# cggos/ptam_cg

Hardware: AMD Instinct MI355X
Metric: BA LM iterations/s (50 KF x 5k pts) [+ tracked frames/s @640x480 in 'tracking'] (higher is better)
Workload: dtype f64

## Files before the change

### ptam_cg_amd/csrc/ba_schur.inc

```
__device__ __forceinline__ void vinv_body(const BaDev& d, double lambda, int bx) {
    const int p = bx * 256 + threadIdx.x;
    if (p >= d.P) return;
    double v[6];
    const int r0 = d.rowptr[p], r1 = d.rowptr[p + 1];
    const int c0 = r0 >> 6, c1 = (r1 - 1) >> 6;
    if (d.cut != nullptr && r1 > r0 && c0 != c1) {
        const double* q = d.cut + (size_t)(2 * c0 + 1) * 9;
        double e[3] = {q[6], q[7], q[8]};
#pragma unroll
        for (int i = 0; i < 6; i++) v[i] = q[i];
        for (int c = c0 + 1; c <= c1; c++) {
            q = d.cut + (size_t)(2 * c) * 9;
#pragma unroll
            for (int i = 0; i < 6; i++) v[i] += q[i];
#pragma unroll
            for (int i = 0; i < 3; i++) e[i] += q[6 + i];
        }
#pragma unroll
        for (int i = 0; i < 3; i++) d.epsB[(size_t)p * 3 + i] = e[i];
    } else {
#pragma unroll
        for (int i = 0; i < 6; i++) v[i] = d.V[(size_t)p * 6 + i];
    }
    double A[9] = {v[0], v[1], v[3], v[1], v[2], v[4], v[3], v[4], v[5]};
    double* out = d.Vinv + (size_t)p * 9;
    if (A[0] * A[4] * A[8] == 0) {
#pragma unroll
        for (int i = 0; i < 9; i++) out[i] = 0;
        return;
    }
    A[0] *= (1.0 + lambda);
    A[4] *= (1.0 + lambda);
    A[8] *= (1.0 + lambda);
    for (int col = 0; col < 3; col++) {
        double inv_diag = 1;
        for (int row = col; row < 3; row++) {
            double val = A[row * 3 + col];
            for (int c2 = 0; c2 < col; c2++) val -= A[c2 * 3 + col] * A[row * 3 + c2];
            if (row == col) {
                A[row * 3 + col] = val;
                inv_diag = 1 / val;
            } else {
                A[col * 3 + row] = val;
                A[row * 3 + col] = val * inv_diag;
            }
        }
    }
    for (int c = 0; c < 3; c++) {
        double y[3], x[3];
        for (int i = 0; i < 3; i++) {
            double val = (i == c) ? 1.0 : 0.0;
            for (int j = 0; j < i; j++) val -= A[i * 3 + j] * y[j];
            y[i] = val;
        }
        for (int i = 0; i < 3; i++) y[i] /= A[i * 3 + i];
        for (int i = 2; i >= 0; i--) {
            double val = y[i];
            for (int j = i + 1; j < 3; j++) val -= A[j * 3 + i] * x[j];
            x[i] = val;
        }
        for (int r = 0; r < 3; r++) out[r * 3 + c] = x[r];
    }
}

__global__ void __launch_bounds__(256) vinv_kernel(BaDev d, double lambda) {
    TL_MARK(d, 6)
    if (ba_guard_blocks(d)) return;
    vinv_body(d, lambda, blockIdx.x);
}
__global__ void __launch_bounds__(256) reduce_vinv_kernel(BaDev d, int grid_acc, int nx, double lambda, double lambda_stay) {
    TL_MARK(d, 5)
    const int4 gf = ba_guard_load(d);
    if (ba_guard_blocks(d, gf)) return;
    if (ba_guard_stay(d, gf)) lambda = lambda_stay;
    const int b = blockIdx.x, nr = nx * RSPLIT;
    if (b < nr)
        reduce_partials_body(d, grid_acc, b % nx, b / nx);
    else
        vinv_body(d, lambda, b - nr);
}

#define SCHUR_TILE_ELEMS (SCHUR_TC * SCHUR_TC * 36 + SCHUR_TC * 6)
#ifndef SCHUR_RING
#define SCHUR_RING 2
#endif
#ifndef SCHUR_NW
#define SCHUR_NW 4
#endif
#define SCHUR_WG_PER_CU (8 / SCHUR_NW)
#define SCHUR_RED_BYTES ((SCHUR_NW / 2) * 40 * 64 * 8)
#define SCHUR_N_VARIANTS 6
#define SCHUR_MAP_WPT 8

struct SchurGrp {
    double wa[3][3];
    double wb[3][3];
    double vi[9];
    double eb[3];
    unsigned pm;
};
typedef double v4f64 __attribute__((ext_vector_type(4)));
typedef double schur_d2 __attribute__((ext_vector_type(2), aligned(8)));

template <int MODE>
__host__ __device__ __forceinline__ int schur_row(int t, int rid) {
    if (MODE == 1) return rid;
    if (t < 2) return 6 * (rid / 3) + 2 * (rid % 3) + t;
    const int q = 16 + (rid >> 1);
    return 6 * (q / 3) + 2 * (q % 3) + (rid & 1);
}
struct SchurLane {
    int hi4, sh4, hi2, sh2;
    unsigned o4, o2;
};
template <int MODE>
__device__ __forceinline__ SchurLane schur_lane(int l15) {
    SchurLane L;
    const int r0 = schur_row<MODE>(0, l15), r2 = MODE == 3 ? schur_row<3>(2, l15) : 0;
    const int s0 = r0 / 6, s2 = r2 / 6;
    L.hi4 = s0 >> 2, L.sh4 = 8 * (s0 & 3), L.o4 = 8u * (unsigned)(r0 - 6 * s0);
    L.hi2 = s2 >> 2, L.sh2 = 8 * (s2 & 3), L.o2 = 8u * (unsigned)(r2 - 6 * s2);
    return L;
}

__device__ __forceinline__ unsigned schur_slot_off(unsigned o0, unsigned o1, int first, int hi, int sh, int M, bool& present) {
    const unsigned o = ((hi ? o1 : o0) >> sh) & 0xffu;
    present = o != 0xffu;
    return (present ? (unsigned)first + o : (unsigned)M) * 48u;
}

template <int MODE>
__device__ __forceinline__ void schur_fetch_role(const char* __restrict__ W0, const char* __restrict__ W1, const char* __restrict__ W2,
                                                 unsigned o0, unsigned o1, int first, const SchurLane& L, int M, double w[3][3],
                                                 bool& pres01, bool& pres2) {
    pres2 = false;
    const unsigned off4 = schur_slot_off(o0, o1, first, L.hi4, L.sh4, M, pres01) + L.o4;
#ifdef SCHUR_NOLOAD
    for (int t = 0; t < 3; t++) w[t][0] = w[t][1] = w[t][2] = (double)off4;
    return;
#endif
    if (MODE == 1) {
        w[0][0] = *(const double*)(W0 + off4);
        w[0][1] = *(const double*)(W1 + off4);
        w[0][2] = *(const double*)(W2 + off4);
        return;
    }
    const double2 p0 = *(const double2*)(W0 + off4), p1 = *(const double2*)(W1 + off4), p2 = *(const double2*)(W2 + off4);
    w[0][0] = p0.x, w[1][0] = p0.y;
    w[0][1] = p1.x, w[1][1] = p1.y;
    w[0][2] = p2.x, w[1][2] = p2.y;
    if (MODE == 3) {
        const unsigned off2 = schur_slot_off(o0, o1, first, L.hi2, L.sh2, M, pres2) + L.o2;
#ifdef SCHUR_NOFRAG2
        w[2][0] = w[2][1] = w[2][2] = (double)off2;
        return;
#endif
        w[2][0] = *(const double*)(W0 + off2);
        w[2][1] = *(const double*)(W1 + off2);
        w[2][2] = *(const double*)(W2 + off2);
    }
}

// ... 315 lines not shown
    std::vector<unsigned> dev((size_t)SCHUR_N_VARIANTS * NT * SCHUR_MAP_WPT, 0xffffffffu);
    for (int v = 0; v < SCHUR_N_VARIANTS; v++)
        for (int t = 0; t < NT; t++)
            for (int i = 0; i < SCHUR_MAP_WPT && t + NT * i < NE2; i++) {
                const int e = t + NT * i;
                dev[((size_t)v * NT + t) * SCHUR_MAP_WPT + i] = (unsigned)m[(size_t)v * SCHUR_TILE_ELEMS + 2 * e] | ((unsigned)m[(size_t)v * SCHUR_TILE_ELEMS + 2 * e + 1] << 16);
            }
    return dev;
}

__global__ void __launch_bounds__(64 * SCHUR_NW) __attribute__((amdgpu_waves_per_eu(2, 2))) schur_tile_mfma_kernel(BaDev d) {
    TL_MARK(d, 7)
    extern __shared__ __attribute__((aligned(16))) double red[];
#ifdef SCHUR_STAMPS
    const long long t_entry = (long long)__builtin_amdgcn_s_memtime();
    if (threadIdx.x == 0 && blockIdx.x < 512) {
        unsigned hw, xcc;
        asm volatile("s_getreg_b32 %0, hwreg(HW_REG_HW_ID)" : "=s"(hw));
        asm volatile("s_getreg_b32 %0, hwreg(HW_REG_XCC_ID)" : "=s"(xcc));
        d.dbg[3072 + 2 * blockIdx.x] = ((long long)__builtin_amdgcn_s_memrealtime() & ((1ll << 40) - 1)) | ((long long)((xcc & 0xf) << 16 | (hw & 0xffff)) << 40);
    }
#endif
#ifdef SCHUR_NO_HEAD
    const int sg0 = d.s_wg_seg[blockIdx.x], sg1 = d.s_wg_seg[blockIdx.x + 1];
#else
    const int4 h0 = ((const int4*)d.s_wg_head)[2 * blockIdx.x], h1 = ((const int4*)d.s_wg_head)[2 * blockIdx.x + 1];
    const int sg0 = h0.x, sg1 = h0.y;
#endif
    for (int sg = sg0; sg < sg1; sg++) {
#ifdef SCHUR_NO_HEAD
        const SchurWG wg = d.s_segs[sg];
#else
        const SchurWG wg = sg == sg0 ? SchurWG{h0.z, h0.w, h1.x, h1.y} : d.s_segs[sg];
#endif
        int a = (int)((sqrt(8.0 * wg.pair + 1.0) - 1.0) * 0.5);
        while ((a + 1) * (a + 2) / 2 <= wg.pair) a++;
        while (a * (a + 1) / 2 > wg.pair) a--;
        const int b = wg.pair - a * (a + 1) / 2;
        const int ncam = min(SCHUR_TC, d.F - a * SCHUR_TC);
        const int ma = ncam <= 2 ? 1 : (ncam <= 5 ? 2 : 3);
        if (a == b) {
            if (ma == 3) schur_tile_body<true, 3, 3>(d, wg, red);
            else if (ma == 2) schur_tile_body<true, 2, 2>(d, wg, red);
            else schur_tile_body<true, 1, 1>(d, wg, red);
        } else {
            if (ma == 3) schur_tile_body<false, 3, 3>(d, wg, red);
            else if (ma == 2) schur_tile_body<false, 2, 3>(d, wg, red);
            else schur_tile_body<false, 1, 3>(d, wg, red);
        }
        __syncthreads();
    }
#ifdef SCHUR_STAMPS
    if (threadIdx.x == 0 && blockIdx.x < 512) d.dbg[3072 + 2 * blockIdx.x + 1] = (long long)__builtin_amdgcn_s_memrealtime() | ((long long)(sg1 - sg0) << 56);
    if ((blockIdx.x == 0 || blockIdx.x == 150) && threadIdx.x == 0) {
        long long* o = d.dbg + 2048 + (blockIdx.x ? 512 : 0) + 264;
        o[0] = t_entry, o[1] = (long long)__builtin_amdgcn_s_memtime(), o[2] = sg1 - sg0;
    }
#endif
}

#define SRED_SLICES 10
__device__ __forceinline__ double schur_sum_partials(const double* __restrict__ elem, int w0, int w1) {
#ifdef SRED_NOLOAD
    return (double)(w1 - w0);
#endif
    double s0 = 0, s1 = 0, s2 = 0, s3 = 0;
    for (int w = w0; w < w1; w += 32) {
        double q[32];
#pragma unroll
        for (int i = 0; i < 32; i++) {
            const double v = elem[(size_t)min(w + i, w1 - 1) * SCHUR_TILE_ELEMS];
            q[i] = w + i < w1 ? v : 0.0;
        }
#pragma unroll
        for (int i = 0; i < 32; i += 4) {
            s0 += q[i];
            s1 += q[i + 1];
            s2 += q[i + 2];
            s3 += q[i + 3];
        }
    }
    return (s0 + s1) + (s2 + s3);
}
__global__ void __launch_bounds__(256) schur_reduce_kernel(BaDev d, double lambda, int pad_identity) {
    TL_MARK(d, 8)
    const int pair = blockIdx.x, slice = blockIdx.y;
    int a = (int)((sqrt(8.0 * pair + 1.0) - 1.0) * 0.5);
    while ((a + 1) * (a + 2) / 2 <= pair) a++;
    while (a * (a + 1) / 2 > pair) a--;
    const int b = pair - a * (a + 1) / 2;
    const int wg0 = d.s_pair_wg_begin[pair], wg1 = d.s_pair_wg_begin[pair + 1];
    double* S = d.SE;
    double* E = se_E(d);
    const int band = se_band(d);
    const size_t FS = (size_t)d.F * 27;
    if (slice < 9) {
        const int idx = slice * 256 + threadIdx.x;
        const int jk = idx / 36, rc = idx - jk * 36;
        const int j = jk >> 3, k = jk & 7, r = rc / 6, c = rc - r * 6;
        const int fa = a * SCHUR_TC + j, fb = b * SCHUR_TC + k;
        if (fa >= d.F || fb >= d.F) return;
        if (a == b && j < k) return;
        const int Rr = 6 * fa + r, Cc = 6 * fb + c, Rb = Rr / SOLVE_NB, Cb = Cc / SOLVE_NB;
        if (Cb > Rb || Rb - Cb > band) return;
        const bool dg = a == b && j == k;
        const int rr = r >= c ? r : c, cc = r >= c ? c : r;
        double uq[RSPLIT];
#pragma unroll
        for (int sp = 0; sp < RSPLIT; sp++) uq[sp] = dg ? d.Usplit[sp * FS + fa * 27 + rr * (rr + 1) / 2 + cc] : 0.0;
        const double tsum = schur_sum_partials(d.s_part + idx, wg0, wg1);
        double val = -tsum;
        if (dg) {
            double u = 0;
#pragma unroll
            for (int sp = 0; sp < RSPLIT; sp++) u += uq[sp];
            if (r == c) u *= (1.0 + lambda);
            val += u;
        }
        S[se_blk(Rb, Cb, band) + (size_t)(Rr % SOLVE_NB) * SOLVE_NB + (Cc % SOLVE_NB)] = val;
        return;
    }
    if (a == b && threadIdx.x < SCHUR_TC * 6) {
        const int idx = threadIdx.x;
        const int j = idx / 6, r = idx - j * 6;
        const int fa = a * SCHUR_TC + j;
        if (fa < d.F) {
            const double s = schur_sum_partials(d.s_part + SCHUR_TC * SCHUR_TC * 36 + idx, wg0, wg1);
            double ea = 0;
#pragma unroll
            for (int sp = 0; sp < RSPLIT; sp++) ea += d.Usplit[sp * FS + fa * 27 + 21 + r];
            E[6 * fa + r] = ea - s;
        }
    }
    {
        const int np = d.npad - d.n, total = np * d.npad;
        for (int idx = pair * 256 + threadIdx.x; idx < total; idx += 256 * (int)gridDim.x) {
            const int q = idx / d.npad;
            const int r = d.n + q, c = idx - q * d.npad;
            const int Rb = r / SOLVE_NB, Cb = c / SOLVE_NB;
            if (c <= r && Rb - Cb <= band)
                S[se_blk(Rb, Cb, band) + (size_t)(r % SOLVE_NB) * SOLVE_NB + (c % SOLVE_NB)] = (r == c && pad_identity) ? 1.0 : 0.0;
        }
    }
    if (pair == 0) {
        const int np = d.npad - d.n;
        for (int idx = threadIdx.x; idx < np; idx += 256) E[d.n + idx] = 0.0;
    }
}
```

### ptam_cg_amd/csrc/bundle.h

```cpp
#pragma once
#include <cstddef>

#include "common.h"

enum { MS_ALIVE = 0, MS_BAD = 1, MS_DEAD = 2 };

#define BA_CHUNK 256
#define SCHUR_TC 8
#define SOLVE_NB 32
#define HIST_BINS 4096

struct BaChunk {
    int pt_begin, pt_end, m_begin, m_end;
};

struct SchurEntry {
    int pt;
    int ma;
    int mb;
    int pad;
    unsigned offa[2];
    unsigned offb[2];
};
struct SchurWG {
    int pair;
    int e_begin, e_end;
    int slot;
};

struct BaScalars {
    double sigma_sq;
    double cur_err;
    double new_err;
    double sumsq_cam;
    double sumsq_pt;
    double median;
    long long n_valid;
    int n_bad;
    int n_outliers;
    int sel_bin;
    int sel_k;
    int n_cand;
    int sel_bin2;
    int sel_k2;
    int select_overflow;
    int n_outliers_pub;
    int pad_;
    int end_step;
    int spec_go;
    int spec_stay;
    int spec_seq;
    int abort_any;
    int solve_fault;
};
static_assert(offsetof(BaScalars, end_step) % 16 == 0 && sizeof(BaScalars) % 8 == 0, "BaScalars: the decision words are read as one 16-byte load");

struct BaDev {
    int C, F, P, M;
    int guard;
    int guard_seq;
    int n, npad;
    int band;
    int n_chunks, grid_acc;
    int u_rows;
    int n_wchunks;
    int n_tiles, n_pairs, n_schur_wg, n_schur_entries;
    double* pose[2];
    int* cam_free;
    double* pt[2];
    double* V;
    double* epsB;
    double* Vinv;
    double* cut;
    int* rowptr;
    int* m_cam;
    int* m_pt;
    double2* m_found;
    double* m_s;
    int* m_orig;
    int* m_fidx;
    uint8_t* m_state;
    double* m_e2;
    double* m_e2t;
    uint8_t* m_zbad_t;
    double* W;
    double* Usplit;
    double* Upart;
    double* Adet;
    int* cam_ptr;
    int* cam_meas;
    double* err_part;
    int* bad_part;
    BaChunk* chunks;
    BaChunk* wchunks;
    unsigned* hist;
    double* cand;
    SchurEntry* s_entries;
    SchurWG* s_segs;
    int* s_wg_seg;
    int* s_pair_wg_begin;
    int* s_wg_head;
    double* s_part;
    unsigned* s_map;
    double* SE;
    double* L;
    double* Dg;
    double* y;
    double* da;
    double *SE2, *L2, *Dg2, *y2;
    unsigned* sflags2;
    unsigned* sflags;
    unsigned solve_seq;
    int chain_off;
    int chain_xcd;
    int spin_limit;
    double* bw_scratch;
    double* sumsq2;
    int* outliers;
    BaScalars* sc;
    long long* dbg;
};

__host__ __device__ __forceinline__ size_t w_plane(const BaDev& d) { return (size_t)(d.M + 1) * 6; }

__host__ __device__ __forceinline__ size_t se_blocks_before_row(int bi, int band) {
    return bi <= band ? (size_t)bi * (bi + 1) / 2 : (size_t)(band + 1) * (band + 2) / 2 + (size_t)(bi - band - 1) * (band + 1);
}
__host__ __device__ __forceinline__ size_t se_blk(int bi, int bj, int band) {
    const int j0 = bi - band > 0 ? bi - band : 0;
    return (se_blocks_before_row(bi, band) + (size_t)(bj - j0)) * (SOLVE_NB * SOLVE_NB);
}
__host__ __device__ __forceinline__ size_t se_size(int nblk, int band) { return se_blocks_before_row(nblk, band) * (SOLVE_NB * SOLVE_NB); }
__host__ __device__ __forceinline__ int se_band(const BaDev& d) {
    const int nblk = d.npad / SOLVE_NB;
    return d.band < nblk - 1 ? d.band : (nblk > 0 ? nblk - 1 : 0);
}
__host__ __device__ __forceinline__ double* se_E(const BaDev& d) { return d.SE + se_size(d.npad / SOLVE_NB, se_band(d)); }

#define MS_LOG 15
#define MS_CH (1 << MS_LOG)
#define MS_CH_BYTES ((size_t)MS_CH * 32)
template <class B>
__host__ __device__ __forceinline__ B* ms_chunk(B* base, size_t i) { return base + (i >> MS_LOG) * MS_CH_BYTES; }
__host__ __device__ __forceinline__ const int& ms_cam(const char* base, size_t i) { return ((const int*)ms_chunk(base, i))[i & (MS_CH - 1)]; }
__host__ __device__ __forceinline__ const int& ms_pt(const char* base, size_t i) { return ((const int*)(ms_chunk(base, i) + (size_t)MS_CH * 4))[i & (MS_CH - 1)]; }
__host__ __device__ __forceinline__ const double2& ms_found(const char* base, size_t i) { return ((const double2*)(ms_chunk(base, i) + (size_t)MS_CH * 8))[i & (MS_CH - 1)]; }
__host__ __device__ __forceinline__ const double& ms_sig(const char* base, size_t i) { return ((const double*)(ms_chunk(base, i) + (size_t)MS_CH * 24))[i & (MS_CH - 1)]; }

struct Carver {
    size_t off = 0;
    size_t take(size_t bytes) {
        const size_t o = off;
        off += (bytes + 255) & ~(size_t)255;
        return o;
    }
// ... 36 lines not shown
```

### ptam_cg_amd/csrc/bundle.hip

```cpp
#include <algorithm>
#include <array>
#include <chrono>
#include <climits>
#include <atomic>
#include <numeric>
#include <utility>

#include "bundle.h"
#include "../../include/ptam_hip_bench.h"

#include "ba_math.inc"
#include "ba_pass1.inc"
#include "ba_select.inc"
#include "ba_jacobian.inc"
#include "ba_schur.inc"
#include "ba_update.inc"
#include "ba_prepare.inc"

template <class T>
struct PinVec {
    ptam_ctx* ctx = nullptr;
    T* p = nullptr;
    size_t n = 0, cap = 0, cap_bytes = 0;
    size_t size() const { return n; }
// ... 365 lines not shown
    const int n_cu = ctx->n_cu > 0 ? ctx->n_cu : 256;
    auto k7_fn = [&](int threads) -> const void* { return k7_wave_fn(threads, ba->k7_loop, ba->opts.estimator, ba->k7_big, ba->det); };
    auto k7_occupancy = [&](int threads, int* per_cu) -> int { return ba_k7_occupancy(ctx, k7_fn(threads), threads, k7_smem(threads), per_cu); };
    int per_cu = 0;
    {
        const size_t lds_max = 160 * 1024;
        if (k7_smem(ba->k7_threads) > lds_max) {
            for (int t : {512, 256})
                if (k7_smem(t) <= lds_max) {
                    ba->k7_threads = t;
                    break;
                }
            if (k7_smem(ba->k7_threads) > lds_max) {
                ba->k7_big = true;
                ba->k7_loop = true;
                ba->k7_threads = 256;
            }
        }
        if (ba->det && !ba->k7_big && ba->k7_threads != (ba->k7_loop ? 256 : 1024)) {
            ba->k7_loop = true;
            ba->k7_threads = 256;
        }
    }
    if (int rc = k7_occupancy(ba->k7_threads, &per_cu)) {
        ptam_set_error("the accumulation kernel cannot be launched with %zu bytes of LDS (%d free cameras)", k7_smem(ba->k7_threads), F);
        return rc;
    }
    if (ba->k7_loop && !ba->k7_big && !ba->det) {
        for (int t : {512, 1024}) {
            int per_cu_t = 0;
            if (int rc = k7_occupancy(t, &per_cu_t)) return rc;
            if (per_cu_t * t > per_cu * ba->k7_threads) {
                ba->k7_threads = t;
                per_cu = per_cu_t;
            }
        }
    }
    per_cu = std::max(1, std::min(per_cu, 8));
    if (ba->use_wave && ba->k7_loop && !ba->k7_big) {
        if (const char* e = ptam_ab_env("PTAM_K7_THREADS")) {
            const int t = atoi(e);
            if ((t == 256 || t == 512 || t == 1024) && !(ba->det && t != 256) && k7_smem(t) <= 160 * 1024) {
                ba->k7_threads = t;
                if (int rc = k7_occupancy(t, &per_cu)) return rc;
                per_cu = std::max(1, std::min(per_cu, 8));
            }
        }
        if (const char* e = ptam_ab_env("PTAM_K7_WG_PER_CU")) per_cu = std::max(1, std::min(per_cu, atoi(e)));
    }
    if (ba->use_wave && !ba->k7_loop) {
        if (const char* e = ptam_ab_env("PTAM_K7_THREADS1")) {
            const int t = atoi(e);
            if ((t == 512 || t == 1024) && !(ba->det && t != 1024) && k7_smem(t) <= 160 * 1024) {
                ba->k7_threads = t;
                if (int rc = k7_occupancy(t, &per_cu)) return rc;
            }
        }
    }
    ba->smem_acc = k7_smem(ba->k7_threads);
    if (ba->use_wave) {
        const int n64 = (M + 63) / 64;
        const int wpb = ba->k7_threads / 64;
        if (ba->k7_loop) {
            d.grid_acc = std::max(1, std::min(n_cu * per_cu, n64 / wpb));
            const int waves = d.grid_acc * wpb;
            ba->per_wave = n64 / waves;
            ba->extra_waves = n64 - ba->per_wave * waves;
        } else {
            ba->per_wave = 1;
            ba->extra_waves = 0;
            d.grid_acc = std::max(1, (n64 + wpb - 1) / wpb);
        }
    } else
        d.grid_acc = 1;
    const int n_dtiles = (M + DET_TILE - 1) / DET_TILE;
    d.u_rows = ba->det ? n_dtiles : (ba->k7_big || !ba->use_wave) ? 1 : d.grid_acc;
    lap("launch shape");

    Carver cv;
    const size_t Mz = std::max(M, 1), Pz = std::max(P_all, 1), Cz = std::max(C, 1), Fz = std::max(F, 1), Maz = std::max(Mall, 1);
    const size_t chunks_cap = std::min<size_t>(Pz, (size_t)M / 64 + (size_t)P_all / 128 + 8);
    const size_t o_pose0 = cv.take(Cz * 96), o_pose1 = cv.take(Cz * 96);
    const size_t o_pt0 = cv.take(Pz * 24), o_pt1 = cv.take(Pz * 24), o_V = cv.take(Pz * 48), o_epsB = cv.take(Pz * 24),
                 o_Vinv = cv.take(Pz * 72), o_rowptr = cv.take((Pz + 1) * 4),
                 o_cut = cv.take(ba->use_wave ? (size_t)((M + 63) / 64) * 2 * 72 : 8);
    const size_t o_mcam = cv.take(Mz * 4), o_mpt = cv.take(Mz * 4), o_mfound = cv.take(Mz * 16), o_ms = cv.take(Mz * 8),
                 o_morig = cv.take(Mz * 4), o_mfidx = cv.take(Mz * 4), o_mstate = cv.take(Mz), o_me2 = cv.take(Mz * 8), o_me2t = cv.take(Mz * 8), o_zbad = cv.take(Mz), o_W = cv.take((Mz + 1) * 144);
    const size_t o_U = cv.take(Fz * 27 * 8 * 16), o_Upart = cv.take((size_t)std::max(d.grid_acc, ba->det ? n_dtiles : 1) * Fz * 27 * 8);
    const size_t o_adet = cv.take(ba->det ? Mz * 14 * 8 : 8), o_camptr = cv.take(ba->det ? (size_t)n_dtiles * (Fz + 1) * 4 : 8), o_cammeas = cv.take(ba->det ? Mz * 4 : 8),
                 o_tilefree = cv.take(ba->det ? ((size_t)n_dtiles + 1) * 4 : 8);
    const size_t n_part = std::max<size_t>(chunks_cap, (size_t)d.grid_acc);
    const size_t o_errp = cv.take(n_part * 16 + 16), o_badp = cv.take((size_t)d.grid_acc * 4 + 16);
    const size_t o_chunks = cv.take(chunks_cap * sizeof(BaChunk));
    const size_t o_wchunks = cv.take(sizeof(BaChunk));
    const size_t o_hist = cv.take(2 * HIST_BINS * 4), o_cand = cv.take(Mz * 8);
    const size_t npad = std::max(d.npad, SOLVE_NB);
    const size_t se_full = se_size((int)(npad / SOLVE_NB), (int)(npad / SOLVE_NB) - 1);
    const size_t o_SE = cv.take((se_full + npad + 8) * 8), o_L = cv.take(se_full * 8), o_Dg = cv.take(npad * 8),
                 o_y = cv.take(npad * 8), o_da = cv.take(npad * 8), o_sq2 = cv.take(16),
                 o_bws = cv.take(npad * 8 * 12), o_sflags = cv.take(ba_solve_flag_bytes((int)(npad / SOLVE_NB))),
                 o_sflags2 = cv.take(ba_solve_flag_bytes((int)(npad / SOLVE_NB))), o_SE2 = cv.take((se_full + npad + 8) * 8),
                 o_L2 = cv.take(se_full * 8), o_Dg2 = cv.take(npad * 8), o_y2 = cv.take(npad * 8);
    const size_t o_out = cv.take(Mz * 4), o_sc = cv.take(sizeof(BaScalars)), o_dbg = cv.take(65536), o_xchg = cv.take(4096);
    const int nw = std::max(1, (n_tiles + 31) / 32);
    const size_t hist_n = (size_t)8 * std::max(n_pairs, 1) * 16;
    const size_t o_cnt = cv.take(Pz * 4), o_tcode = cv.take(Pz * (size_t)nw * 8), o_phist = cv.take(hist_n * 4);
    const size_t clear_bytes = cv.off;
    Carver sm;
    const size_t s_ps = sm.take(sizeof(PrepScalars)), s_pose = sm.take(Cz * 96), s_camfree = sm.take(Cz * 4),
                 s_porder = sm.take(pair_order.size() * 4);
    const size_t o_small = cv.take(sm.off);
    const size_t o_rdead = cv.take(Maz), o_ptsraw = cv.take(Pz * 24);
    const size_t o_start = cv.take((Pz + 1) * 4), o_denseof = cv.take(Pz * 4), o_ptorig = cv.take(Pz * 4), o_arr = cv.take(Maz * 4),
                 o_tmpi = cv.take(Mz * 4), o_tmpkey = cv.take(Mz * 4), o_ptile = cv.take(Mz * 16), o_kp = cv.take(Pz * 4),
                 o_costp = cv.take(Pz * 4), o_entpre = cv.take((Pz + 1) * 8), o_costpre = cv.take((Pz + 1) * 8), o_ebase = cv.take(hist_n * 4);
    ba->block_bytes = cv.off;
    if (!ctx_cache_take(ctx->dev_cache, CTX_NCACHE(ctx->dev_cache), ba->block_bytes, &ba->block, &ba->block_cap)) {
        HIP_TRY(hipMalloc(&ba->block, ba->block_bytes));
        ba->block_cap = ba->block_bytes;
    }
    HIP_TRY(hipMemsetAsync(ba->block, 0, clear_bytes, ctx->stream));
    char* base = (char*)ba->block;
    d.pose[0] = (double*)(base + o_small + s_pose);
    d.pose[1] = (double*)(base + o_pose1);
    (void)o_pose0;
    d.cam_free = (int*)(base + o_small + s_camfree);
    d.pt[0] = (double*)(base + o_pt0);
    d.pt[1] = (double*)(base + o_pt1);
    d.V = (double*)(base + o_V);
    d.epsB = (double*)(base + o_epsB);
    d.Vinv = (double*)(base + o_Vinv);
    d.cut = ba->use_wave ? (double*)(base + o_cut) : nullptr;
    d.rowptr = (int*)(base + o_rowptr);
    d.m_cam = (int*)(base + o_mcam);
    d.m_pt = (int*)(base + o_mpt);
    d.m_found = (double2*)(base + o_mfound);
    d.m_s = (double*)(base + o_ms);
    d.m_orig = (int*)(base + o_morig);
    d.m_fidx = (int*)(base + o_mfidx);
    d.m_state = (uint8_t*)(base + o_mstate);
    d.m_e2 = (double*)(base + o_me2);
    d.m_e2t = (double*)(base + o_me2t);
    d.m_zbad_t = (uint8_t*)(base + o_zbad);
    d.W = (double*)(base + o_W);
    d.Usplit = (double*)(base + o_U);
    d.Upart = (double*)(base + o_Upart);
    d.Adet = ba->det ? (double*)(base + o_adet) : nullptr;
    d.cam_ptr = (int*)(base + o_camptr);
    d.cam_meas = (int*)(base + o_cammeas);
    d.err_part = (double*)(base + o_errp);
    d.bad_part = (int*)(base + o_badp);
    d.chunks = (BaChunk*)(base + o_chunks);
    d.wchunks = (BaChunk*)(base + o_wchunks);
    d.hist = (unsigned*)(base + o_hist);
    d.cand = (double*)(base + o_cand);
    d.SE = (double*)(base + o_SE);
    d.L = (double*)(base + o_L);
    d.Dg = (double*)(base + o_Dg);
    d.y = (double*)(base + o_y);
    d.da = (double*)(base + o_da);
    d.sumsq2 = (double*)(base + o_sq2);
    d.bw_scratch = (double*)(base + o_bws);
    d.sflags = (unsigned*)(base + o_sflags);
    d.sflags2 = (unsigned*)(base + o_sflags2);
    d.SE2 = (double*)(base + o_SE2);
    d.L2 = (double*)(base + o_L2);
    d.Dg2 = (double*)(base + o_Dg2);
    d.y2 = (double*)(base + o_y2);
    d.solve_seq = 0;
    d.chain_off = 0;
    {
        static std::atomic<unsigned> next_xcd{0};
        d.chain_xcd = (int)(next_xcd.fetch_add(1) & 7u);
        static const int lim = [] {
            const char* e = getenv("PTAM_CH_SPIN_LIMIT");
            return e ? std::max(1, atoi(e)) : CH_SPIN_DEFAULT;
        }();
        d.spin_limit = lim;
    }
    d.outliers = (int*)(base + o_out);
    d.sc = (BaScalars*)(base + o_sc);
    d.dbg = (long long*)(base + o_dbg);
    ba->d_xchg = (double*)(base + o_xchg);
    if (!ctx->d_smap) {
        static const std::vector<unsigned> s_map = schur_index_map_device();
        HIP_TRY(hipMalloc((void**)&ctx->d_smap, s_map.size() * 4));
        HIP_TRY(hipMemcpy(ctx->d_smap, s_map.data(), s_map.size() * 4, hipMemcpyHostToDevice));
    }
    d.s_map = ctx->d_smap;
    lap("alloc + clear");

    Carver hs;
    const size_t h_stamp = hs.take(64), h_psrb = hs.take(sizeof(PrepScalars)), h_rowptr = hs.take((Pz + 1) * 4), h_ptorig = hs.take(Pz * 4),
                 h_small = hs.take(sm.off), h_chunks = hs.take(chunks_cap * sizeof(BaChunk)), h_dead = hs.take(ba->n_dead > 0 ? Maz : 1);
    (void)h_stamp;
    void* pin = nullptr;
    {
        const size_t later = 64 + (size_t)C * 96 + (size_t)P_all * 24 + (size_t)M * 4 + 64;
        const int rc_p = ctx_pinned(ctx, std::max(hs.off, later), &pin);
        if (rc_p) return rc_p;
    }
    char* hp = (char*)pin;
    char* dp = (char*)ctx->d_pinned;
    volatile unsigned long long* stamp = (volatile unsigned long long*)hp;
    PrepScalars* ps_host = (PrepScalars*)(hp + h_psrb);
    {
        PrepScalars init;
        std::memset(&init, 0, sizeof init);
        init.dup_key = ~0ull;
        std::memcpy(hp + h_small + s_ps, &init, sizeof init);
        std::memcpy(hp + h_small + s_pose, ba->cam_pose.data(), (size_t)C * 96);
        std::memcpy(hp + h_small + s_camfree, cam_free.data(), (size_t)C * 4);
        std::memcpy(hp + h_small + s_porder, pair_order.data(), pair_order.size() * 4);
    }
// ... 341 lines not shown
        }
        HIP_TRY(hipMemsetAsync(ba->d_gather, 0, (size_t)total * 8, ctx->stream));
        if (n_local > 0)
            hipLaunchKernelGGL(place_keys_kernel, dim3((n_local + 255) / 256), dim3(256), 0, ctx->stream,
                               (const double*)d.cand, n_local, ba->d_gather + off);
        rc = ba_allreduce(ba, ba->d_gather, (size_t)total);
        if (rc) return rc;
        BaDev dg = d;
        dg.cand = ba->d_gather + ba->gather_cap;
        if (total > 0)
            hipLaunchKernelGGL(hist_keys_kernel, dim3((int)std::max<long long>(1, std::min<long long>((total + 255) / 256, 1024))),
                               dim3(256), 0, ctx->stream, (const double*)ba->d_gather, total, d.hist);
        hipLaunchKernelGGL(select_compact_kernel, dim3((int)std::max<long long>(1, std::min<long long>((total + 1023) / 1024, 256))),
                           dim3(256), 0, ctx->stream, dg, (const double*)ba->d_gather, total, (const uint8_t*)nullptr, 0);
        hipLaunchKernelGGL(select_final_kernel, dim3(1), dim3(1024), 0, ctx->stream, dg, ba->opts.estimator, min_s2);
        prof_end(ba, PTAM_K_SELECT);
        HIP_TRY(hipGetLastError());
        return PTAM_OK;
    }
    hipLaunchKernelGGL(select_final_kernel, dim3(1), dim3(1024), 0, ctx->stream, d, ba->opts.estimator, min_s2);
    prof_end(ba, PTAM_K_SELECT);
    HIP_TRY(hipGetLastError());
    return PTAM_OK;
}

static void launch_k7(ptam_ba* ba, int guard = 0) {
    ptam_ctx* ctx = ba->ctx;
    BaDev d = ba->d;
    d.guard = guard;
    d.guard_seq = (int)ba->mbox_seq;
    int cur = guard ? (ba->cur ^ 1) : ba->cur;
    if ((ba->k7_big && !ba->det) || !ba->use_wave)
        (void)hipMemsetAsync(d.Upart, 0, std::max<size_t>(1, (size_t)d.F * 27) * sizeof(double), ctx->stream);
    if (!ba->use_wave) {
        (void)hipMemsetAsync(d.err_part, 0, 16, ctx->stream);
        (void)hipMemsetAsync(d.bad_part, 0, 4, ctx->stream);
        return;
    }
    int est = ba->opts.estimator;
    void* args[] = {&ctx->cam, &d, &cur, &est, &ba->per_wave, &ba->extra_waves};
    (void)hipLaunchKernel(k7_wave_fn(ba->k7_threads, ba->k7_loop, est, ba->k7_big, ba->det), dim3(d.grid_acc), dim3(ba->k7_threads), args,
                          ba->smem_acc, ctx->stream);
    if (ba->det && d.F > 0)
        hipLaunchKernelGGL(reduce_det_kernel, dim3(d.u_rows), dim3(256), (size_t)14 * (DET_TILE + 1) * sizeof(double), ctx->stream, d);
}

static int ba_pass2(ptam_ba* ba) {
    ptam_ctx* ctx = ba->ctx;
    BaDev& d = ba->d;
    prof_begin(ba, PTAM_K_JACOBIAN);
    launch_k7(ba);
    prof_end(ba, PTAM_K_JACOBIAN);
    hipLaunchKernelGGL(reduce_partials_kernel, dim3(std::max(1, (d.F * 27 + 63) / 64), RSPLIT), dim3(256), 0, ctx->stream,
                       d, d.grid_acc);
    HIP_TRY(hipGetLastError());
    if (ba->comm && ba->world > 1) {
        if (d.F > 0) {
            hipLaunchKernelGGL(pack2_kernel, dim3(1), dim3(1), 0, ctx->stream, (const BaScalars*)d.sc, se_E(d) + d.npad, 0, 0);
            ba->cur_pending = true;
        } else {
            hipLaunchKernelGGL(pack2_kernel, dim3(1), dim3(1), 0, ctx->stream, (const BaScalars*)d.sc, ba->d_xchg, 0, 0);
            int rc = ba_allreduce(ba, ba->d_xchg, 2);
            if (rc) return rc;
            hipLaunchKernelGGL(unpack2_kernel, dim3(1), dim3(1), 0, ctx->stream, d.sc, (const double*)ba->d_xchg, 0);
        }
    }
    return PTAM_OK;
}

static int ba_ensure_mailbox(ptam_ba* ba) {
    if (ba->mbox) return PTAM_OK;
    void* h = nullptr;
    size_t cap = 0;
    if (!ctx_cache_take(ba->ctx->host_cache, CTX_NCACHE(ba->ctx->host_cache), sizeof(ptam_ba::Mailbox), &h, &cap))
        HIP_TRY(hipHostMalloc(&h, sizeof(ptam_ba::Mailbox), hipHostMallocMapped | hipHostMallocCoherent));
    std::memset(h, 0, sizeof(ptam_ba::Mailbox));
    void* dv = nullptr;
    HIP_TRY(hipHostGetDevicePointer(&dv, h, 0));
    ba->mbox = (ptam_ba::Mailbox*)h;
    ba->mbox_dev = (ptam_ba::Mailbox*)dv;
    return PTAM_OK;
}

static int ba_trial(ptam_ba* ba, double lambda, bool skip_vinv, int last_allowed, int abort_local, bool decide_in_prologue = false) {
    ptam_ctx* ctx = ba->ctx;
    BaDev& d = ba->d;
    prof_begin(ba, PTAM_K_VINV);
    if (d.P > 0 && !skip_vinv) hipLaunchKernelGGL(vinv_kernel, dim3((d.P + 255) / 256), dim3(256), 0, ctx->stream, d, lambda);
    prof_end(ba, PTAM_K_VINV);
    if (d.F > 0) {
        prof_begin(ba, PTAM_K_SCHUR);
        if (d.n_schur_wg > 0)
            hipLaunchKernelGGL(schur_tile_mfma_kernel, dim3(d.n_schur_wg), dim3(64 * SCHUR_NW), SCHUR_RED_BYTES, ctx->stream, d);
        hipLaunchKernelGGL(schur_reduce_kernel, dim3(d.n_pairs, SRED_SLICES), dim3(256), 0, ctx->stream, d, lambda,
                           (ba->world > 1 && ba->rank != 0) ? 0 : 1);
        prof_end(ba, PTAM_K_SCHUR);
        HIP_TRY(hipGetLastError());
        const size_t n_se = se_size(d.npad / SOLVE_NB, se_band(d)) + d.npad;
        const bool sharded = ba->comm && ba->world > 1;
        if (sharded) prof_begin(ba, PTAM_K_EXCHANGE);
        int rc = ba_allreduce(ba, d.SE, n_se + (ba->cur_pending ? 2 : 0));
        if (sharded) prof_end(ba, PTAM_K_EXCHANGE);
        if (rc) return rc;
        if (ba->cur_pending) {
            hipLaunchKernelGGL(unpack2_kernel, dim3(1), dim3(1), 0, ctx->stream, d.sc, (const double*)(d.SE + n_se), 0);
            ba->cur_pending = false;
        }
        prof_begin(ba, PTAM_K_SOLVE);
        rc = ba_solve(ctx, d, ba->cur);
        prof_end(ba, PTAM_K_SOLVE);
        if (rc) return rc;
    }
    prof_begin(ba, PTAM_K_UPDATE);
    if (d.F == 0)
        hipLaunchKernelGGL(pose_update_kernel, dim3(std::max(1, (d.C + 63) / 64)), dim3(64), 0, ctx->stream, d, ba->cur);
    if (d.n_chunks > 0)
        hipLaunchKernelGGL(point_update_kernel, dim3(d.n_chunks), dim3(BA_CHUNK), 0, ctx->stream, ctx->cam, d, ba->cur,
                           ba->opts.estimator);
    {
        const bool fuse = !(ba->comm && ba->world > 1) && !ba->prof;
        ulonglong2* slots = nullptr;
        unsigned long long seq = 0;
        if (fuse) {
            const int rcm = ba_ensure_mailbox(ba);
            if (rcm) return rcm;
            slots = (ulonglong2*)ba->mbox_dev;
            seq = ++ba->mbox_seq;
            ba->published_by_finalize = true;
        }
        ba->decide_pending = decide_in_prologue;
        ba->decide_last_allowed = last_allowed;
        if (!decide_in_prologue)
            hipLaunchKernelGGL(finalize_new_kernel, dim3(1), dim3(256), 0, ctx->stream, d, ba->opts.update_sq_conv_limit, last_allowed,
                               slots, seq);
    }
    prof_end(ba, PTAM_K_UPDATE);
    HIP_TRY(hipGetLastError());
    if (ba->comm && ba->world > 1) {
        hipLaunchKernelGGL(pack2_kernel, dim3(1), dim3(1), 0, ctx->stream, (const BaScalars*)d.sc, ba->d_xchg, 1, abort_local);
        int rc = ba_allreduce(ba, ba->d_xchg, 4);
        if (rc) return rc;
        hipLaunchKernelGGL(unpack2_kernel, dim3(1), dim3(1), 0, ctx->stream, d.sc, (const double*)ba->d_xchg, 1);
    }
    return PTAM_OK;
}

static int ba_p1_blocks() {
    static const int n = [] {
        const char* e = ptam_ab_env("PTAM_P1_BLOCKS");
        return e ? std::max(1, atoi(e)) : 512;
    }();
    return n;
}
static int ba_enqueue_speculative(ptam_ba* ba, double lambda_next, double lambda_stay) {
    ptam_ctx* ctx = ba->ctx;
    BaDev d = ba->d;
    const double min_s2 = ba->opts.min_sigma * ba->opts.min_sigma;
    d.guard = 1;
    d.guard_seq = (int)ba->mbox_seq;
    const dim3 g_p1(std::max(1, std::min((d.M + 256 * P1_U - 1) / (256 * P1_U), ba_p1_blocks())));
    if (ba->decide_pending) {
        hipLaunchKernelGGL(purge_pass1_decide_kernel, g_p1, dim3(256), 0, ctx->stream, d, ba->opts.update_sq_conv_limit, ba->decide_last_allowed,
                           (ulonglong2*)ba->mbox_dev, ba->mbox_seq);
        ba->decide_pending = false;
    } else
        hipLaunchKernelGGL(purge_pass1_kernel, g_p1, dim3(256), 0, ctx->stream, d);
    hipLaunchKernelGGL(select_compact_kernel, dim3(std::max(1, std::min((d.M + 1023) / 1024, ba_sel_blocks()))), dim3(256), 0, ctx->stream, d,
                       (const double*)d.m_e2, (long long)d.M, (const uint8_t*)d.m_state, 0);
    hipLaunchKernelGGL(select_final_kernel, dim3(1), dim3(1024), 0, ctx->stream, d, ba->opts.estimator, min_s2);
    launch_k7(ba, 1);
    {
        const int nx = std::max(1, (d.F * 27 + 63) / 64);
        hipLaunchKernelGGL(reduce_vinv_kernel, dim3(nx * RSPLIT + (d.P + 255) / 256), dim3(256), 0, ctx->stream, d, d.grid_acc, nx,
                           lambda_next, lambda_stay);
    }
    HIP_TRY(hipGetLastError());
    return PTAM_OK;
}
// ... 359 lines not shown
        }
        ba->ev_ok = true;
    }
    ba->prof = on != 0;
    return PTAM_OK;
}

int ptam_ba_kernel_time(const ptam_ba* ba, int kernel, double* total_ms, int* launches) {
    ARG_TRY(ba && kernel >= 0 && kernel < PTAM_K_COUNT);
    if (total_ms) *total_ms = ba->k_ms[kernel];
    if (launches) *launches = ba->k_n[kernel];
    return PTAM_OK;
}

int ptam_ba_set_comm(ptam_ba* ba, int rank, int world, ptam_allreduce_f64_fn fn, void* user) {
    ARG_TRY(ba && world >= 1 && rank >= 0 && rank < world);
    ARG_TRY(world == 1 || fn);
    ARG_TRY(world <= 32);
    if (ba->d_sel && world != ba->world) {
        HIP_TRY(hipSetDevice(ba->ctx->device));
        HIP_TRY(ptam_stream_wait(ba->ctx->stream));
        HIP_TRY(hipFree(ba->d_sel));
        ba->d_sel = nullptr;
    }
    ba->rank = rank;
    ba->world = world;
    ba->comm = fn;
    ba->comm_user = user;
    return PTAM_OK;
}

#define BA_DBG(...) do { if (dbg.wait) { std::fprintf(stderr, "[ptam] " __VA_ARGS__); std::fprintf(stderr, "\n"); } } while (0)
int ptam_ba_compute(ptam_ba* ba, const volatile unsigned char* abort_flag, int* accepted_out) {
    ARG_TRY(ba);
    ptam_ctx* ctx = ba->ctx;
    const BaDebug& dbg = ba_debug();
    HIP_TRY(hipSetDevice(ctx->device));
    BA_DBG("compute: prepare");
    const bool sharded = ba->comm && ba->world > 1;
    int rc = ptam_ba_prepare(ba);
    if (rc && !sharded) return rc;
    const int rc_prepare = rc;
    BA_DBG("compute: prepared M=%d P=%d F=%d chunks=%d wchunks=%d grid_acc=%d schur_wg=%d", ba->d.M, ba->d.P, ba->d.F, ba->d.n_chunks,
           ba->d.n_wchunks, ba->d.grid_acc, ba->d.n_schur_wg);
    BaDev& d = ba->d;
    ChainTurn chain_turn(d, ctx->device);
    double lambda = 0.0001, lambda_factor = 2.0;
    ba->converged = ba->published_by_finalize = ba->cur_pending = ba->slow_select = false;
    ba->trial_is_current = ba->e2_is_current = false;
    bool hit_max = false;
    int counter = 0;
    ba->accepted = 0;
    ba->trials.clear();
    std::vector<int> step_outlier_end;
    int n_steps = 0;
    bool prev_end_pending = false;
    bool abort_all = false;
    auto abort_local = [&]() { return abort_flag && *abort_flag; };
    auto aborted = [&]() { return sharded ? abort_all : abort_local(); };
    BaScalars sc;
    std::memset(&sc, 0, sizeof sc);
    double dbg_enq_ms = 0, dbg_wait_ms = 0;
    std::vector<double> trial_read_us;
    const auto dbg_t0 = std::chrono::steady_clock::now();
    BaHostTimes ht;
    ba_dbg_begin(ba, ht);
    if (sharded && (rc = ba_sharded_handshake(ba, rc_prepare, abort_local(), &abort_all, chain_turn))) return rc;
    const bool empty = d.M == 0;
    const bool spec = !sharded && !ba->prof && d.n_chunks > 0 && !ptam_ab_env("PTAM_NO_SPECULATION");
    bool spec_ready = false;
    const bool fused_decision = !ptam_ab_env("PTAM_SEPARATE_FINALIZE");
    while (!empty && !ba->converged && !hit_max && !aborted()) {
        bool skip_vinv = false;
        if (spec_ready) {
            spec_ready = false;
            skip_vinv = true;
        } else {
            if ((rc = ba_pass1_sigma(ba))) return rc;
            if ((rc = ba_pass2(ba))) return rc;
        }
        bool have_cur = false;
        double cur_err = 0, new_err = 0;
        bool ran_any = false, redo_step = false, nan_stop = false;
        for (;;) {
            if (have_cur && !(new_err > cur_err)) break;
            if (ba->converged || hit_max || aborted()) break;
            BA_DBG("trial %d lambda %g", counter, lambda);
            const auto q0 = std::chrono::steady_clock::now();
            rc = ba_trial(ba, lambda, skip_vinv, counter + 1 >= ba->opts.max_iterations ? 1 : 0, abort_local() ? 1 : 0, spec && fused_decision);
            dbg_enq_ms += ba_stall_ms(q0, counter, "took", "to enqueue");
            skip_vinv = false;
            if (rc) return rc;
            if ((rc = ba_publish_scalars(ba))) return rc;
            if (spec) {
                if ((rc = ba_enqueue_speculative(ba, lambda * 0.3, lambda))) return rc;
            }
            BA_DBG("trial %d enqueued, waiting", counter);
            const auto w0 = std::chrono::steady_clock::now();
            rc = ba_wait_scalars(ba, &sc);
            dbg_wait_ms += ba_stall_ms(w0, counter, "waited", "for its scalars");
            if (rc) return rc;
            BA_DBG("trial %d read: cur %g new %g sigma2 %g median %g n_valid %lld n_bad %d sumsq %g %g", counter, sc.cur_err, sc.new_err,
                   sc.sigma_sq, sc.median, sc.n_valid, sc.n_bad, sc.sumsq_cam, sc.sumsq_pt);
            ba_dbg_first_read(ht);
            if (!have_cur) {
                if (prev_end_pending) step_outlier_end.push_back(spec && fused_decision ? sc.n_outliers_pub : sc.n_outliers);
                prev_end_pending = false;
                if (sc.select_overflow && !ba->slow_select) {
                    ba->slow_select = true;
                    if (dbg.select) std::fprintf(stderr, "[ptam] rank %d: select overflow, repeating the step on the gather path\n", ba->rank);
                    redo_step = true;
                    break;
                }
                have_cur = true;
                cur_err = sc.cur_err;
                new_err = cur_err + 9999;
                if (!(new_err > cur_err)) {
                    nan_stop = true;
                    break;
                }
            }
            if (sc.solve_fault) {
                if ((rc = ba_solve_fallback(ba, counter))) return rc;
                continue;
            }
            ran_any = true;
            if (dbg.trial_times) trial_read_us.push_back(std::chrono::duration<double, std::micro>(std::chrono::steady_clock::now() - dbg_t0).count());
            if (sharded) abort_all = abort_all || sc.abort_any != 0;
            new_err = sc.new_err;
            const double sumsq = sc.sumsq_cam + sc.sumsq_pt;
            if (sumsq < ba->opts.update_sq_conv_limit) ba->converged = true;
            ptam_ba_trial t;
            t.lambda = lambda;
            t.sigma_sq = sc.sigma_sq;
            t.err_old = cur_err;
            t.err_new = new_err;
            t.sum_sq_update = sumsq;
            t.n_bad = sc.n_bad;
            t.accepted = 0;
            if (ba->opts.verbose)
                std::printf("L%.1e\tOld %.6f  New %.6f  Diff %.6f\n", lambda, cur_err, new_err, cur_err - new_err);
            if (new_err > cur_err) {
                lambda = lambda * lambda_factor;
                lambda_factor = lambda_factor * 2;
            }
            counter++;
            if (counter >= ba->opts.max_iterations) hit_max = true;
            ba->trials.push_back(t);
        }
        if (redo_step) continue;
        if (nan_stop) hit_max = true;
        ba->trial_is_current = false;
        ba->e2_is_current = ran_any && !(new_err < cur_err);
        if (ran_any && new_err < cur_err) {
            lambda_factor = 2.0;
            lambda *= 0.3;
            ba->cur ^= 1;
            ba->accepted++;
            ba->trials.back().accepted = 1;
            ba->trial_is_current = true;
        }
        if (prev_end_pending) {
            if ((rc = ba_read_scalars(ba, &sc))) return rc;
            step_outlier_end.push_back(sc.n_outliers);
        }
        const bool stayed = spec && ran_any && !(new_err < cur_err) && !(new_err > cur_err) && !ba->converged && !hit_max;
        spec_ready = (spec && ran_any && new_err < cur_err && !ba->converged && !hit_max) || stayed;
        if (!spec_ready && d.M > 0)
            hipLaunchKernelGGL(purge_kernel, dim3((d.M + 255) / 256), dim3(256), 0, ctx->stream, d);
        prev_end_pending = true;
        HIP_TRY(hipGetLastError());
        n_steps++;
    }
    BA_DBG("loop done, steps %d", n_steps);
    ba_report_trial_times(ba, trial_read_us);
    if (dbg.stall)
        std::fprintf(stderr, "[ptam] compute loop: %zu trials in %.3f ms; host enqueueing trials %.3f ms, waiting for scalars %.3f ms\n",
                     ba->trials.size(), std::chrono::duration<double, std::milli>(std::chrono::steady_clock::now() - dbg_t0).count(),
                     dbg_enq_ms, dbg_wait_ms);
    if (n_steps > 0) {
        if ((rc = ba_read_scalars(ba, &sc))) return rc;
        step_outlier_end.push_back(sc.n_outliers);
    }
    if ((rc = ba_dbg_loop_end(ba, ht))) return rc;
    const int n_out = step_outlier_end.empty() ? 0 : step_outlier_end.back();
    std::vector<int> out_idx(std::max(n_out, 1));
    if ((rc = ba_readback(ba, n_out, out_idx))) return rc;
    ba->raw_out.insert(ba->raw_out.end(), out_idx.begin(), out_idx.begin() + n_out);
    for (int end : step_outlier_end) ba->raw_out_ends.push_back(ba->raw_out_base + end);
    ba->raw_out_base += n_out;
    if (n_out > 0) ba->prepared = false;
    if ((rc = ba_dbg_dump(ba, ht))) return rc;
    if (dbg.stall)
        std::fprintf(stderr, "[ptam] compute total %.3f ms\n",
                     std::chrono::duration<double, std::milli>(std::chrono::steady_clock::now() - dbg_t0).count());
    if (accepted_out) *accepted_out = ba->accepted;
    return PTAM_OK;
}

int ptam_ba_converged(const ptam_ba* ba) { return ba && ba->converged ? 1 : 0; }

int ptam_ba_get_point(const ptam_ba* ba, int n, double pos[3]) {
    ARG_TRY(ba && pos && n >= 0 && n < (int)(ba->pts.size() / 3));
    std::memcpy(pos, &ba->pts[3 * (size_t)n], 24);
    return PTAM_OK;
}
int ptam_ba_get_camera(const ptam_ba* ba, int n, double pose[12]) {
    ARG_TRY(ba && pose && n >= 0 && n < (int)ba->cam_fixed.size());
    std::memcpy(pose, &ba->cam_pose[12 * (size_t)n], 96);
    return PTAM_OK;
}
int ptam_ba_get_all(const ptam_ba* ba, double* poses12, double* points3) {
    ARG_TRY(ba);
    if (poses12) std::memcpy(poses12, ba->cam_pose.data(), ba->cam_pose.size() * 8);
    if (points3) std::memcpy(points3, ba->pts.data(), ba->pts.size() * 8);
    return PTAM_OK;
}
int ptam_ba_get_outliers(const ptam_ba* ba, int32_t* pairs, int cap) {
    if (!ba) return PTAM_E_ARG;
    ba_finish_outliers(const_cast<ptam_ba*>(ba));
    const int n = (int)ba->outliers.size();
    for (int i = 0; i < n && i < cap && pairs; i++) {
        pairs[2 * i] = ba->outliers[i].first;
        pairs[2 * i + 1] = ba->outliers[i].second;
    }
    return n;
}
// ... 205 lines not shown
```

Measured before the change: 6381.

## Speculatively compute retry-lambda Vinv inside schur_reduce for rejected LM steps

Adds extra grid rows to schur_reduce_kernel that compute the point-block inverses for the next retry lambda (lambda*factor) into a second buffer, Vinv_alt. When a trial is rejected, the host swaps Vinv and Vinv_alt and skips the vinv kernel launch on the retry. This removes one kernel launch and its dependency from the rejected-step path. In exchange every trial does the extra inverse work and uses more memory, and the rows touching epsB may race with or duplicate other writes.

```diff
diff --git a/ptam_cg_amd/csrc/ba_schur.inc b/ptam_cg_amd/csrc/ba_schur.inc
--- a/ptam_cg_amd/csrc/ba_schur.inc
+++ b/ptam_cg_amd/csrc/ba_schur.inc
@@ -1,4 +1,4 @@
-__device__ __forceinline__ void vinv_body(const BaDev& d, double lambda, int bx) {
+__device__ __forceinline__ void vinv_body(const BaDev& d, double lambda, int bx, double* __restrict__ vinv) {
     const int p = bx * 256 + threadIdx.x;
     if (p >= d.P) return;
     double v[6];
@@ -23,7 +23,7 @@
         for (int i = 0; i < 6; i++) v[i] = d.V[(size_t)p * 6 + i];
     }
     double A[9] = {v[0], v[1], v[3], v[1], v[2], v[4], v[3], v[4], v[5]};
-    double* out = d.Vinv + (size_t)p * 9;
+    double* out = vinv + (size_t)p * 9;
     if (A[0] * A[4] * A[8] == 0) {
 #pragma unroll
         for (int i = 0; i < 9; i++) out[i] = 0;
@@ -66,7 +66,7 @@
 __global__ void __launch_bounds__(256) vinv_kernel(BaDev d, double lambda) {
     TL_MARK(d, 6)
     if (ba_guard_blocks(d)) return;
-    vinv_body(d, lambda, blockIdx.x);
+    vinv_body(d, lambda, blockIdx.x, d.Vinv);
 }
 __global__ void __launch_bounds__(256) reduce_vinv_kernel(BaDev d, int grid_acc, int nx, double lambda, double lambda_stay) {
     TL_MARK(d, 5)
@@ -77,7 +77,7 @@
     if (b < nr)
         reduce_partials_body(d, grid_acc, b % nx, b / nx);
     else
-        vinv_body(d, lambda, b - nr);
+        vinv_body(d, lambda, b - nr, d.Vinv);
 }
 
 #define SCHUR_TILE_ELEMS (SCHUR_TC * SCHUR_TC * 36 + SCHUR_TC * 6)
@@ -559,9 +559,13 @@
     }
     return (s0 + s1) + (s2 + s3);
 }
-__global__ void __launch_bounds__(256) schur_reduce_kernel(BaDev d, double lambda, int pad_identity) {
+__global__ void __launch_bounds__(256) schur_reduce_kernel(BaDev d, double lambda, int pad_identity, double lambda_retry) {
     TL_MARK(d, 8)
     const int pair = blockIdx.x, slice = blockIdx.y;
+    if (slice >= SRED_SLICES) {
+        vinv_body(d, lambda_retry, (slice - SRED_SLICES) * (int)gridDim.x + pair, d.Vinv_alt);
+        return;
+    }
     int a = (int)((sqrt(8.0 * pair + 1.0) - 1.0) * 0.5);
     while ((a + 1) * (a + 2) / 2 <= pair) a++;
     while (a * (a + 1) / 2 > pair) a--;
diff --git a/ptam_cg_amd/csrc/bundle.h b/ptam_cg_amd/csrc/bundle.h
--- a/ptam_cg_amd/csrc/bundle.h
+++ b/ptam_cg_amd/csrc/bundle.h
@@ -71,6 +71,7 @@
     double* V;
     double* epsB;
     double* Vinv;
+    double* Vinv_alt;
     double* cut;
     int* rowptr;
     int* m_cam;
diff --git a/ptam_cg_amd/csrc/bundle.hip b/ptam_cg_amd/csrc/bundle.hip
--- a/ptam_cg_amd/csrc/bundle.hip
+++ b/ptam_cg_amd/csrc/bundle.hip
@@ -471,7 +471,7 @@
     const size_t chunks_cap = std::min<size_t>(Pz, (size_t)M / 64 + (size_t)P_all / 128 + 8);
     const size_t o_pose0 = cv.take(Cz * 96), o_pose1 = cv.take(Cz * 96);
     const size_t o_pt0 = cv.take(Pz * 24), o_pt1 = cv.take(Pz * 24), o_V = cv.take(Pz * 48), o_epsB = cv.take(Pz * 24),
-                 o_Vinv = cv.take(Pz * 72), o_rowptr = cv.take((Pz + 1) * 4),
+                 o_Vinv = cv.take(Pz * 72), o_Vinv2 = cv.take(Pz * 72), o_rowptr = cv.take((Pz + 1) * 4),
                  o_cut = cv.take(ba->use_wave ? (size_t)((M + 63) / 64) * 2 * 72 : 8);
     const size_t o_mcam = cv.take(Mz * 4), o_mpt = cv.take(Mz * 4), o_mfound = cv.take(Mz * 16), o_ms = cv.take(Mz * 8),
                  o_morig = cv.take(Mz * 4), o_mfidx = cv.take(Mz * 4), o_mstate = cv.take(Mz), o_me2 = cv.take(Mz * 8), o_me2t = cv.take(Mz * 8), o_zbad = cv.take(Mz), o_W = cv.take((Mz + 1) * 144);
@@ -519,6 +519,7 @@
     d.V = (double*)(base + o_V);
     d.epsB = (double*)(base + o_epsB);
     d.Vinv = (double*)(base + o_Vinv);
+    d.Vinv_alt = (double*)(base + o_Vinv2);
     d.cut = ba->use_wave ? (double*)(base + o_cut) : nullptr;
     d.rowptr = (int*)(base + o_rowptr);
     d.m_cam = (int*)(base + o_mcam);
@@ -1026,9 +1027,11 @@
     return PTAM_OK;
 }
 
-static int ba_trial(ptam_ba* ba, double lambda, bool skip_vinv, int last_allowed, int abort_local, bool decide_in_prologue = false) {
+static int ba_trial(ptam_ba* ba, double lambda, double lambda_retry, bool skip_vinv, int last_allowed, int abort_local, bool decide_in_prologue,
+                    bool* alt_written) {
     ptam_ctx* ctx = ba->ctx;
     BaDev& d = ba->d;
+    *alt_written = false;
     prof_begin(ba, PTAM_K_VINV);
     if (d.P > 0 && !skip_vinv) hipLaunchKernelGGL(vinv_kernel, dim3((d.P + 255) / 256), dim3(256), 0, ctx->stream, d, lambda);
     prof_end(ba, PTAM_K_VINV);
@@ -1036,8 +1039,11 @@
         prof_begin(ba, PTAM_K_SCHUR);
         if (d.n_schur_wg > 0)
             hipLaunchKernelGGL(schur_tile_mfma_kernel, dim3(d.n_schur_wg), dim3(64 * SCHUR_NW), SCHUR_RED_BYTES, ctx->stream, d);
-        hipLaunchKernelGGL(schur_reduce_kernel, dim3(d.n_pairs, SRED_SLICES), dim3(256), 0, ctx->stream, d, lambda,
-                           (ba->world > 1 && ba->rank != 0) ? 0 : 1);
+        const bool alt = !(ba->comm && ba->world > 1) && !ba->prof && d.P > 0 && d.n_pairs > 0;
+        const int vinv_rows = alt ? ((d.P + 255) / 256 + d.n_pairs - 1) / d.n_pairs : 0;
+        hipLaunchKernelGGL(schur_reduce_kernel, dim3(d.n_pairs, SRED_SLICES + vinv_rows), dim3(256), 0, ctx->stream, d, lambda,
+                           (ba->world > 1 && ba->rank != 0) ? 0 : 1, lambda_retry);
+        *alt_written = alt;
         prof_end(ba, PTAM_K_SCHUR);
         HIP_TRY(hipGetLastError());
         const size_t n_se = se_size(d.npad / SOLVE_NB, se_band(d)) + d.npad;
@@ -1563,12 +1569,20 @@
         bool have_cur = false;
         double cur_err = 0, new_err = 0;
         bool ran_any = false, redo_step = false, nan_stop = false;
+        bool retry_from_alt = false;
         for (;;) {
             if (have_cur && !(new_err > cur_err)) break;
             if (ba->converged || hit_max || aborted()) break;
             BA_DBG("trial %d lambda %g", counter, lambda);
             const auto q0 = std::chrono::steady_clock::now();
-            rc = ba_trial(ba, lambda, skip_vinv, counter + 1 >= ba->opts.max_iterations ? 1 : 0, abort_local() ? 1 : 0, spec && fused_decision);
+            if (retry_from_alt) {
+                std::swap(d.Vinv, d.Vinv_alt);
+                retry_from_alt = false;
+                skip_vinv = true;
+            }
+            bool alt_written = false;
+            rc = ba_trial(ba, lambda, lambda * lambda_factor, skip_vinv, counter + 1 >= ba->opts.max_iterations ? 1 : 0, abort_local() ? 1 : 0,
+                          spec && fused_decision, &alt_written);
             dbg_enq_ms += ba_stall_ms(q0, counter, "took", "to enqueue");
             skip_vinv = false;
             if (rc) return rc;
@@ -1624,6 +1638,7 @@
             if (new_err > cur_err) {
                 lambda = lambda * lambda_factor;
                 lambda_factor = lambda_factor * 2;
+                retry_from_alt = alt_written;
             }
             counter++;
             if (counter >= ba->opts.max_iterations) hit_max = true;
```

Measured after the change: 6335. About the same (-0.7%).
